# boqian333/E2ENet-Medical

Hardware: AMD Instinct MI355X
Metric: voxels/sec (train step fwd+bwd+update), 128^3 patch 32ch density=0.2 (higher is better)
Workload: dtype f32 (fp16x2 split products, f32 accumulate); 1 GPU; BraTS-shaped 4-modal 128^3 patches, shiftConvPP base 32, K=4, DSFF density 0.2, batch 2 per GPU, fwd+loss+bwd+clip+SGD+mask step, dense (parity) wgrad; parallelism=dp1

## Files before the change

e2enet_medical_amd/_lib.py:

```python
import ctypes as C
import os

_HERE = os.path.dirname(os.path.abspath(__file__))
LIB_PATH = os.environ.get("E2E_LIB_PATH") or os.path.join(_HERE, "csrc", "libe2e_hip.so")

KNOWN_ENV = frozenset({
    "E2E_CONV_MM", "E2E_MM_GRID", "E2E_MM_GEOM", "E2E_MM_PAIRQ", "E2E_CONV_DENSE", "E2E_CONV_SPARSE2", "E2E_CONV_PERSIST", "E2E_CONV_WGS",
    "E2E_CONV_KSPLIT", "E2E_WG_H2", "E2E_WG_BF3", "E2E_CT_BF3", "E2E_CT_H2",
    "E2E_CONV_DBG", "E2E_MM_STAMPS",
    "E2E_LIB_PATH", "E2E_STRICT_ENV", "E2E_DENSE_MIN_DENSITY", "E2E_MM_MIN_DENSITY", "E2E_WGRAD_STREAM", "E2E_LANES", "E2E_GRAPHS",
    "E2E_GRAPH_MAX_VOXELS", "E2E_PLAN_CACHE_GB", "E2E_SW_BLOCKING", "E2E_FORCE_DIST",
    "E2E_CPU_THREADS", "E2E_BENCH_DRY", "E2E_BENCH_DRY_FAIL_RANK", "E2E_BENCH_ALL_LAUNCHES",
})


def check_env(environ=None, strict=None):
    environ = os.environ if environ is None else environ
    unknown = sorted(k for k in environ if k.startswith("E2E_") and k not in KNOWN_ENV)
    if not unknown:
        return
    msg = ("unknown E2E_* environment variable(s) %s: not read by this build (known: %s)"
           % (", ".join(unknown), ", ".join(sorted(KNOWN_ENV))))
    if strict is None:
        strict = environ.get("E2E_STRICT_ENV") == "1"
    if strict:
        raise RuntimeError(msg)
    import warnings
    warnings.warn(msg + "; set E2E_STRICT_ENV=1 to refuse instead", RuntimeWarning, stacklevel=2)


class InChan(C.Structure):
    _fields_ = [("ptr", C.c_void_p), ("scale", C.c_void_p), ("shift", C.c_void_p),
                ("nstride", C.c_longlong), ("ab_nstride", C.c_int), ("dshift", C.c_int),
                ("slope", C.c_float), ("reserved", C.c_int)]


class OutChan(C.Structure):
    _fields_ = [("ptr", C.c_void_p), ("nstride", C.c_longlong), ("dshift", C.c_int), ("accumulate", C.c_int)]


class InSumChan(C.Structure):
    _fields_ = [("y", C.c_void_p), ("scale", C.c_void_p), ("shift", C.c_void_p), ("mean", C.c_void_p), ("rstd", C.c_void_p),
                ("part", C.c_void_p), ("nstride", C.c_longlong), ("part_nstride", C.c_longlong), ("ab_nstride", C.c_int),
                ("slope", C.c_float)]
# ... 33 lines not shown
    "e2e_last_error": (C.c_char_p, []),
    "e2e_abi_version": (I, []),
    "e2e_last_kernel": (C.c_char_p, []),
    "e2e_conv133_num_partials": (I, [I, I, I, I, I]),
    "e2e_conv133_fwd": (I, [P, I, P, P, P, P, P, I, I, I, I, I, I, I, I, P]),
    "e2e_conv133_fwd_ws_bytes": (LL, [I, I, I, I, I, I, I, I, I]),
    "e2e_conv133_fwd_splitk": (I, [P, I, P, P, P, P, P, I, I, I, I, I, I, I, I, P, LL, P]),
    "e2e_conv133_dgrad": (I, [P, P, P, P, I, I, I, I, I, I, I, I, I, P]),
    "e2e_conv133_dgrad_ws_bytes": (LL, [I, I, I, I, I, I, I, I, I]),
    "e2e_conv133_dgrad_splitk": (I, [P, P, P, P, I, I, I, I, I, I, I, I, I, P, LL, P]),
    "e2e_conv133_dense_ws_bytes": (LL, [I, I, I, I, I, I, I, I, I]),
    "e2e_conv133_sparse_eligible": (I, [I, I, I, I, I, I, I, I]),
    "e2e_conv133_sparse_wpk_floats": (LL, [I, I, I]),
    "e2e_conv133_sparse_plan": (I, [P, I, I, I, P, P, P, P, P, P]),
    "e2e_conv133_sparse_pack": (I, [P, I, LL, P]),
    "e2e_conv133_fwd_sparse": (I, [P, I, P, P, P, P, I, P, I, P, P, I, I, I, I, I, P]),
    "e2e_conv133_dgrad_sparse": (I, [P, P, P, P, I, P, P, P, I, I, I, I, I, I, I, P]),
    "e2e_conv133_fwd_dense": (I, [P, I, P, P, P, P, P, I, I, I, I, I, P, LL, P]),
    "e2e_conv133_mm_ws_bytes": (LL, [I, I, I, I, I, I, I, I, I]),
    "e2e_conv133_mm_pack": (I, [P, I, LL, P]),
    "e2e_conv133_input_ranges_ws_bytes": (LL, [I]),
    "e2e_conv133_input_ranges": (I, [P, I, P, P]),
    "e2e_absmax_word": (I, [P, LL, P, P]),
    "e2e_conv133_fwd_mm": (I, [P, I, P, P, P, P, P, P, I, I, I, I, I, P]),
    "e2e_conv133_dgrad_mm": (I, [P, P, P, P, P, I, I, I, I, I, I, P]),
    "e2e_conv133_dgrad_dense": (I, [P, P, P, P, I, I, I, I, I, I, P, LL, P]),
    "e2e_conv133_wgrad_ws_bytes": (LL, [I, I, I, I, I, I, I, I, I]),
    "e2e_conv133_wgrad": (I, [P, P, P, P, I, I, I, I, I, I, I, I, I, P, P, P]),
    "e2e_diag_split_gemm": (I, [P, P, P, I, I, P, P]),
    "e2e_diag_kernel_clock": (I, [I, P, P, I]),
    "e2e_in_stats_finalize": (I, [P, I, P, P, F, P, P, P, P, I, I, P]),
    "e2e_in_lrelu_bwd_ws_doubles": (LL, [I, I]),
    "e2e_in_lrelu_bwd": (I, [P, P, P, P, P, P, P, F, P, P, P, P, I, I, LL, P, I, P, P]),
    "e2e_convT_fwd": (I, [P, P, P, F, P, P, P, I, I, I, I, I, I, I, I, I, P, P, P]),
    "e2e_convT_dgrad": (I, [P, P, P, P, I, I, I, I, I, I, I, I, I, I, P, P, P, P]),
    "e2e_convT_wgrad_ws_bytes": (LL, [I, I, I, I, I, I, I, I, I]),
    "e2e_convT_wgrad": (I, [P, P, P, F, P, P, P, I, I, I, I, I, I, I, I, I, P, P, P, P]),
    "e2e_maxpool_fwd": (I, [P, P, P, F, P, I, I, I, I, I, I, I, I, P]),
    "e2e_maxpool_bwd_num_records": (I, [I, I, I, I, I, I]),
    "e2e_maxpool_bwd": (I, [P, P, P, F, P, P, I, I, I, I, I, I, I, I, I, P, P, P, P]),
    "e2e_head1x1_fwd": (I, [P, P, P, F, P, P, I, I, I, LL, P]),
    "e2e_head1x1_dgrad": (I, [P, P, P, I, I, I, I, LL, P]),
    "e2e_head1x1_wgrad_ws_bytes": (LL, [I, I, I, LL]),
    "e2e_head1x1_wgrad": (I, [P, P, P, F, P, P, P, I, I, I, LL, P]),
    "e2e_loss_ws_bytes": (LL, [I, I]),
    "e2e_dc_ce_reduce": (I, [P, P, P, I, I, LL, P]),
    "e2e_dc_ce_grad": (I, [P, P, P, F, I, F, P, P, I, I, LL, P]),
    "e2e_dc_ce_fold_batch": (I, [P, I, I, P]),
    "e2e_online_eval_counts": (I, [P, P, P, I, I, LL, P]),
    "e2e_dc_bce_reduce": (I, [P, P, P, P, I, I, LL, P]),
    "e2e_dc_bce_grad": (I, [P, P, P, P, F, I, F, P, P, I, I, LL, P]),
    "e2e_online_eval_regions": (I, [P, P, P, P, I, I, LL, P]),
    "e2e_seg_to_regions": (I, [P, P, P, I, I, LL, P]),
    "e2e_ds_target_gather": (I, [P, P, P, P, P, I, I, I, I, I, I, I, P]),
    "e2e_grad_sqnorm": (I, [P, I, P, P]),
    "e2e_sgd_clip_mask_step": (I, [P, I, P, F, F, F, F, I, I, P]),
    "e2e_apply_mask": (I, [P, I, P]),
    "e2e_dsff_kernel_l1": (I, [P, P, I, I, I, I, I, P]),
    "e2e_dsff_kth_value": (I, [P, I, I, P, P, P]),
    "e2e_dsff_death": (I, [P, P, P, I, P]),
    "e2e_dsff_grad_score": (I, [P, P, F, P, P, I, I, I, I, I, P]),
    "e2e_dsff_grow_above": (I, [P, P, P, I, I, I, P]),
    "e2e_dsff_expand": (I, [P, P, P, P, I, I, I, P]),
    "e2e_dsff_expand_quads": (I, [P, P, P, I, I, P]),
    "e2e_dsff_kmask_from_weights": (I, [P, P, I, I, I, P]),
    "e2e_flip3d": (I, [P, P, I, I, I, I, I, P]),
# ... 25 lines not shown


class _Lib:
    def __init__(self, path):
        if not os.path.exists(path):
            raise ImportError(
                "libe2e_hip.so not found at %s: build it with `python -c 'import __graft_entry__ as g; g.build()'` "
                "or `make -C e2enet_medical_amd/csrc`. There is no CPU fallback." % path)
        self._dll = C.CDLL(path)
        self.path = path
        for name, (res, args) in SIGNATURES.items():
            fn = getattr(self._dll, name)
            fn.restype = res
            fn.argtypes = args
            if name in _NO_STATUS:
                setattr(self, name[4:], fn)
            else:
                setattr(self, name[4:], self._checked(name, fn))

    def _checked(self, name, fn):
        last_error = self._dll.e2e_last_error

        def call(*a):
            rc = fn(*a)
            if rc != 0:
                raise E2EError("%s failed (%d): %s" % (name, rc, (last_error() or b"").decode()))
        call.__name__ = name
        return call


_lib = None


ABI_VERSION = 19


def lib() -> _Lib:
    global _lib
    if _lib is None:
        import torch
        check_env()
        handle = _Lib(LIB_PATH)
        got = handle.abi_version()
        if got != ABI_VERSION:
            raise ImportError("%s reports ABI version %d, this package needs %d: rebuild with `make -C %s`"
                              % (LIB_PATH, got, ABI_VERSION, os.path.dirname(LIB_PATH)))
        _lib = handle
    return _lib
```

e2enet_medical_amd/csrc/api.hip:

```cpp
#include "e2e_common.h"
#include <cstring>

namespace e2e {
static thread_local char g_err[512] = "";
void set_error(const char* fmt, ...) {
  va_list ap;
  va_start(ap, fmt);
  vsnprintf(g_err, sizeof(g_err), fmt, ap);
  va_end(ap);
}
static thread_local char g_kernel[160] = "";
void note_kernel(const char* fmt, ...) {
  va_list ap;
  va_start(ap, fmt);
  vsnprintf(g_kernel, sizeof(g_kernel), fmt, ap);
  va_end(ap);
}
}

extern "C" const char* e2e_last_error(void) { return e2e::g_err; }
extern "C" const char* e2e_last_kernel(void) { return e2e::g_kernel; }
extern "C" int e2e_abi_version(void) { return 19; }

extern "C" int e2e_diag_kernel_clock(int family, double* mhz, double* busy_ms, int reset) {
  E2E_REQUIRE(mhz != nullptr && (family == 0 || family == 1), "diag_kernel_clock: family 0 (conv133_mm) or 1 (conv133_wgrad v5)");
  if (hipDeviceSynchronize() != hipSuccess) return e2e::check_launch("diag_kernel_clock");
  unsigned long long v[2] = {0, 0};
  if (family == 0) e2e::mm_clock_read(v, reset != 0); else e2e::wgrad_clock_read(v, reset != 0);
  *mhz = v[1] ? 100.0 * (double)v[0] / (double)v[1] : 0.0;
  if (busy_ms) *busy_ms = (double)v[1] / 1e5;
  return e2e::check_launch("diag_kernel_clock");
}
```

e2enet_medical_amd/csrc/instnorm.hip:

```cpp
#include "e2e_common.h"
#include "e2e_split.h"

namespace {

struct Stat {
  double n, mean, m2;
};
__device__ __forceinline__ Stat combine(const Stat a, const Stat b) {
  if (b.n == 0.0) return a;
  if (a.n == 0.0) return b;
  Stat r;
  r.n = a.n + b.n;
  const double delta = b.mean - a.mean;
  r.mean = a.mean + delta * (b.n / r.n);
  r.m2 = a.m2 + b.m2 + delta * delta * (a.n * b.n / r.n);
  return r;
}

__global__ __launch_bounds__(256) void in_finalize_kernel(const double* __restrict__ part, int np,
                                                          const float* __restrict__ gamma,
                                                          const float* __restrict__ beta, float eps,
                                                          float* __restrict__ scale, float* __restrict__ shift,
                                                          float* __restrict__ mean_out, float* __restrict__ rstd_out,
                                                          int C) {
// ... 219 lines not shown
  const int c = blockIdx.x;
  double s3 = 0.0;
  if (dbias != nullptr) {
    for (int n = 0; n < B; ++n) {
      const double* q = rec3 + ((long long)n * C + c) * nblocks;
      for (int b = threadIdx.x; b < nblocks; b += 64) s3 += q[b];
    }
    s3 = e2e::wave_sum_d(s3);
  }
  if (threadIdx.x != 0) return;
  double s1 = 0.0, s2 = 0.0;
  for (int n = 0; n < B; ++n) {
    const double* r = sums + ((long long)n * C + c) * 3;
    s1 += r[0];
    s2 += r[1];
  }
  dbeta[c] = (float)s1;
  dgamma[c] = (float)s2;
  if (dbias) dbias[c] = (float)s3;
}

__global__ __launch_bounds__(64) void in_bwd_tile_sums_kernel(const double* __restrict__ part, double* __restrict__ sums, int np,
                                                              unsigned* __restrict__ absmax) {
  const int nc = blockIdx.x;
  if (absmax != nullptr && nc == 0 && threadIdx.x == 0) *absmax = 0u;
  const double* p = part + (long long)nc * np * 2;
  double a = 0.0, b = 0.0;
  for (int i = threadIdx.x; i < np; i += 64) { a += p[2 * i]; b += p[2 * i + 1]; }
  a = e2e::wave_sum_d(a);
  b = e2e::wave_sum_d(b);
  if (threadIdx.x == 0) { sums[(long long)nc * 3] = a; sums[(long long)nc * 3 + 1] = b; sums[(long long)nc * 3 + 2] = 0.0; }
}

}

extern "C" int e2e_in_stats_finalize(const double* part, int np, const float* gamma, const float* beta, float eps,
                                     float* scale, float* shift, float* mean, float* rstd, int B, int C,
                                     void* stream) {
  E2E_REQUIRE(part && gamma && beta && scale && shift && mean && rstd, "in_stats_finalize: null pointer");
  E2E_REQUIRE(np > 0 && B > 0 && C > 0, "in_stats_finalize: bad dims");
  hipLaunchKernelGGL(in_finalize_kernel, dim3(B * C), dim3(256), 0, (hipStream_t)stream, part, np, gamma, beta, eps,
                     scale, shift, mean, rstd, C);
  return e2e::check_launch("in_finalize_kernel");
}

extern "C" long long e2e_in_lrelu_bwd_ws_doubles(int B, int C) { return (long long)B * C * (3 + 3 * 256) + 2; }

extern "C" int e2e_in_lrelu_bwd(float* dz_dy, const float* y, const float* mean, const float* rstd, const float* scale,
                                const float* shift, const float* gamma, float slope, float* dgamma, float* dbeta,
                                float* dbias, float* sums, int B, int C, long long spatial, const double* tile_sums, int np,
                                unsigned* dy_absmax, void* stream) {
  E2E_REQUIRE(dz_dy && y && mean && rstd && scale && shift && gamma && dgamma && dbeta && sums, "in_lrelu_bwd: null pointer");
  E2E_REQUIRE(B > 0 && C > 0 && spatial > 0, "in_lrelu_bwd: bad dims");
  hipStream_t st = (hipStream_t)stream;
  double* ds = reinterpret_cast<double*>(sums);
  double* recs = ds + (long long)B * C * 3;
  double* rec3 = recs + (long long)B * C * 256 * 2;
  long long blocks = e2e::cdivll(spatial, 256 * 4 * 4);
  if (blocks > 256) blocks = 256;
  if (blocks < 1) blocks = 1;
  dim3 grid((unsigned)blocks, B * C);
  if (tile_sums == nullptr) {
    hipLaunchKernelGGL(in_bwd_reduce_kernel, grid, dim3(256), 0, st, dz_dy, y, mean, rstd, scale, shift, slope, recs, C,
                       spatial, dy_absmax, ds);
    hipLaunchKernelGGL(in_bwd_apply_kernel, grid, dim3(256), 0, st, dz_dy, y, mean, rstd, scale, shift, gamma, slope, ds,
                       (const double*)recs, (int)blocks, B, C, spatial, dy_absmax, rec3);
  } else {
    E2E_REQUIRE(np > 0, "in_lrelu_bwd: tile_sums without a record count");
    hipLaunchKernelGGL(in_bwd_tile_sums_kernel, dim3(B * C), dim3(64), 0, st, tile_sums, ds, np, dy_absmax);
    hipLaunchKernelGGL(in_bwd_apply_kernel, grid, dim3(256), 0, st, dz_dy, y, mean, rstd, scale, shift, gamma, slope, ds,
                       (const double*)nullptr, 0, B, C, spatial, dy_absmax, rec3);
  }
  hipLaunchKernelGGL(in_bwd_params_kernel, dim3(C), dim3(64), 0, st, (const double*)ds, (const double*)rec3, (int)blocks,
                     dgamma, dbeta, dbias, B, C);
  return e2e::check_launch("in_lrelu_bwd");
}
```

e2enet_medical_amd/engine.py:

```python
import contextlib
import ctypes as C
import math
import os
from typing import Dict, List, Optional, Sequence, Tuple

import torch

import numpy as np

from ._lib import lib, InChan, OutChan, ParamEntry, SparsePackJob, InSumChan, MmPackJob, RangeSrc, RangeJob

LRELU_SLOPE = 0.01
IN_EPS = 1e-5
DENSE_MIN_DENSITY = float(os.environ.get("E2E_DENSE_MIN_DENSITY", "0.5"))
WGRAD_STREAM = os.environ.get("E2E_WGRAD_STREAM", "1") != "0"
WGRAD_STREAM_MAX_ELEMS = 40000000
WGRAD_LATE = True
LANES = os.environ.get("E2E_LANES", "1") != "0"
LANE_DIVS = None


def _lane_divs(voxels):
    if LANE_DIVS is not None:
        return LANE_DIVS
    return (8, 512) if voxels <= (1 << 20) else (64,)
FUSE_IN_SUMS = 1
SPARSE2 = os.environ.get("E2E_CONV_SPARSE2", "1") != "0"
DENSE_ENABLED = True
MM_FORWARD = MM_BACKWARD = True
MM_MIN_DENSITY = float(os.environ.get("E2E_MM_MIN_DENSITY", "0.125"))


PARAM_EPOCH = 0


def note_native_param_write():
    global PARAM_EPOCH
    PARAM_EPOCH += 1


def shift_amounts(num_channels: int, shift_size: int = 5):
    group = math.ceil(num_channels / shift_size)
    pad = shift_size // 2
    return [c // group - pad for c in range(num_channels)]


def _stream():
    return torch.cuda.current_stream().cuda_stream


@contextlib.contextmanager
def _wgrad_stream(eng, elems):
    side = getattr(eng, "_wg_active", None)
    if side is None or elems > WGRAD_STREAM_MAX_ELEMS:
        yield eng.wgrad_ws
        return
    side.wait_stream(torch.cuda.current_stream())
    with torch.cuda.stream(side):
        yield eng.wgrad_ws_side


def _ptr(t: Optional[torch.Tensor]) -> int:
    return 0 if t is None else t.data_ptr()


def _upload_structs(structs, device) -> torch.Tensor:
    raw = b"".join(bytes(s) for s in structs)
    return torch.frombuffer(bytearray(raw), dtype=torch.uint8).to(device)


class Act:

    def __init__(self, name, shape, normed, device):
        self.name = name
        self.shape = tuple(int(v) for v in shape)
        self.normed = normed
        self.data = torch.empty(self.shape, dtype=torch.float32, device=device)
        b, c = self.shape[:2]
        if normed:
            self.scale = torch.empty(b * c, dtype=torch.float32, device=device)
            self.shift = torch.empty(b * c, dtype=torch.float32, device=device)
            self.mean = torch.empty(b * c, dtype=torch.float32, device=device)
            self.rstd = torch.empty(b * c, dtype=torch.float32, device=device)
        else:
            self.scale = self.shift = self.mean = self.rstd = None
        self.grad: Optional[torch.Tensor] = None
        self.needs_grad = True
        self._grad_written = False
        self.producer = None
        self.last_writer = None
        self.sums_ready = False

    @property
    def spatial(self):
        return self.shape[2] * self.shape[3] * self.shape[4]

    def alloc_grad(self):
        if self.grad is None and self.needs_grad:
            self.grad = torch.empty(self.shape, dtype=torch.float32, device=self.data.device)

    def claim_grad_write(self, op=None) -> int:
        acc = 1 if self._grad_written else 0
        self._grad_written = True
        self.last_writer = op
        return acc


class SparsePlan:

    def __init__(self, km_host, transpose, device):
        L = lib()
        r, cc = km_host.shape
        self.Q, self.P = (cc, r) if transpose else (r, cc)
        self.groups, self.nchunks = (self.Q + 31) // 32, (self.P + 7) // 8
        qslot = np.empty(self.groups * 32, dtype=np.int32)
        pslot = np.empty(self.groups * self.nchunks * 8, dtype=np.int32)
        quads = np.empty(self.groups * 8 * self.nchunks, dtype=np.uint32)
        woff = np.empty(self.groups * self.nchunks * 8, dtype=np.int32)
        flush, kmax = C.c_int(1), C.c_int(1)
        km_host = np.ascontiguousarray(km_host, dtype=np.uint8)
        L.conv133_sparse_plan(km_host.ctypes.data, r, cc, 1 if transpose else 0, qslot.ctypes.data, pslot.ctypes.data,
                              quads.ctypes.data, woff.ctypes.data, C.addressof(kmax), C.addressof(flush))
        self.flush_every, self.kmax = int(flush.value), int(kmax.value)
        self.woff = torch.from_numpy(woff).to(device)
# ... 225 lines not shown
        elif self.use_dense():
            L.conv133_fwd_dense(self.chans.data_ptr(), self.cin, p[self.w_name].data_ptr(), p[self.prefix + ".conv.bias"].data_ptr(),
                                _ptr(self.live), self.out.data.data_ptr(), self.part.data_ptr(), b, self.cout, di, hi, wi, ws.data_ptr(),
                                ws.numel() * 4, _stream())
        elif self.sp_fwd is not None:
            sp = self.sp_fwd
            L.conv133_fwd_sparse(sp.table.data_ptr(), self.cin, sp.wpk.data_ptr(), p[self.prefix + ".conv.bias"].data_ptr(),
                                 sp.quads.data_ptr(), sp.woff.data_ptr(), sp.kmax, sp.qslot.data_ptr(), sp.flush_every, self.out.data.data_ptr(),
                                 self.part.data_ptr(), b, self.cout, di, hi, wi, _stream())
        elif ws is not None and self.fwd_ws_bytes > 0:
            L.conv133_fwd_splitk(self.chans.data_ptr(), self.cin, p[self.w_name].data_ptr(),
                                 p[self.prefix + ".conv.bias"].data_ptr(), _ptr(self.live), self.out.data.data_ptr(),
                                 self.part.data_ptr(), b, self.cout, di, hi, wi, sd, sh, sw, ws.data_ptr(), ws.numel() * 4,
                                 _stream())
        else:
            L.conv133_fwd(self.chans.data_ptr(), self.cin, p[self.w_name].data_ptr(), p[self.prefix + ".conv.bias"].data_ptr(),
                          _ptr(self.live), self.out.data.data_ptr(), self.part.data_ptr(), b, self.cout, di, hi, wi,
                          sd, sh, sw, _stream())
        L.in_stats_finalize(self.part.data_ptr(), self.np, p[self.prefix + ".instnorm.weight"].data_ptr(),
                            p[self.prefix + ".instnorm.bias"].data_ptr(), IN_EPS, self.out.scale.data_ptr(),
                            self.out.shift.data_ptr(), self.out.mean.data_ptr(), self.out.rstd.data_ptr(), b,
                            self.cout, _stream())

    def backward(self):
        e = self.eng
        p, g = e.params, e.grads
        o = self.out
        b = o.shape[0]
        di, hi, wi = self.in_dims
        sd, sh, sw = self.stride
        L = lib()
        ready = o.sums_ready
        o.sums_ready = False
        L.in_lrelu_bwd(o.grad.data_ptr(), o.data.data_ptr(), o.mean.data_ptr(), o.rstd.data_ptr(), o.scale.data_ptr(), o.shift.data_ptr(),
                       p[self.prefix + ".instnorm.weight"].data_ptr(),
                       LRELU_SLOPE, g[self.prefix + ".instnorm.weight"].data_ptr(),
                       g[self.prefix + ".instnorm.bias"].data_ptr(), g[self.prefix + ".conv.bias"].data_ptr(),
                       e.in_sums.data_ptr(), b, self.cout, o.spatial, self.own_sums.data_ptr() if ready else None, self.own_np,
                       self.dy_absmax.data_ptr(), _stream())
        late = WGRAD_LATE and getattr(e, "_wg_active", None) is not None and o.data.numel() > WGRAD_STREAM_MAX_ELEMS
        if not late:
            self._wgrad(e, L, g, o, b, di, hi, wi, sd, sh, sw, o.data.numel())
        if self.do_dgrad:
            ws = getattr(e, "fwd_ws", None)
            if self.use_mm("b"):
                if not hasattr(e, "_refresh_weight_caches"):
                    self.pack_mm_standalone("b")
                L.conv133_dgrad_mm(o.grad.data_ptr(), self.dy_absmax.data_ptr(), self.wpk_bwd.data_ptr(), self.w_absmax.data_ptr(),
                                   self.outs.data_ptr(), b, self.cin, self.cout, di, hi, wi, _stream())
            elif self.use_dense():
                L.conv133_dgrad_dense(o.grad.data_ptr(), p[self.w_name].data_ptr(), _ptr(self.live_t), self.outs.data_ptr(), b, self.cin, self.cout,
                                      di, hi, wi, ws.data_ptr(), ws.numel() * 4, _stream())
            elif self.sp_bwd is not None:
                sp = self.sp_bwd
                table = self._bwd_table()
                L.conv133_dgrad_sparse(o.grad.data_ptr(), sp.wpk.data_ptr(), sp.quads.data_ptr(), sp.woff.data_ptr(), sp.kmax, sp.pslot.data_ptr(),
                                       table.data_ptr(), _ptr(sp.insum), sp.flush_every, b, self.cin, self.cout, di, hi, wi, _stream())
                for s in sp.fused_srcs:
                    s.sums_ready = True
            elif ws is not None and self.dgrad_ws_bytes > 0:
                L.conv133_dgrad_splitk(o.grad.data_ptr(), p[self.w_name].data_ptr(), _ptr(self.live_t), self.outs.data_ptr(),
                                       b, self.cin, self.cout, di, hi, wi, sd, sh, sw, ws.data_ptr(), ws.numel() * 4, _stream())
            else:
                L.conv133_dgrad(o.grad.data_ptr(), p[self.w_name].data_ptr(), _ptr(self.live_t), self.outs.data_ptr(),
                                b, self.cin, self.cout, di, hi, wi, sd, sh, sw, _stream())
        if late:
            self._wgrad(e, L, g, o, b, di, hi, wi, sd, sh, sw, 0)

    def _wgrad(self, e, L, g, o, b, di, hi, wi, sd, sh, sw, elems):
        with _wgrad_stream(e, elems) as ws:
            L.conv133_wgrad(self.chans.data_ptr(), o.grad.data_ptr(), g[self.w_name].data_ptr(), ws.data_ptr(),
                            b, self.cin, self.cout, di, hi, wi, sd, sh, sw, self.dy_absmax.data_ptr(), self.x_absmax_ptr(), _stream())
# ... 111 lines not shown
        self.out.pool_of = src.producer if src.normed else None
        self.acc = 0

    def plan_backward(self):
        self.src.alloc_grad()
        self.acc = self.src.claim_grad_write(self)

    def forward(self):
        s = self.src
        b, c, d, h, w = s.shape
        lib().maxpool_fwd(s.data.data_ptr(), _ptr(s.scale), _ptr(s.shift), LRELU_SLOPE, self.out.data.data_ptr(),
                          b, c, d, h, w, *self.kernel, _stream())

    def backward(self):
        s = self.src
        b, c, d, h, w = s.shape
        fuse = FUSE_IN_SUMS >= 1 and s.normed and s.last_writer is self and s.producer is not None and s.producer.own_sums is not None
        lib().maxpool_bwd(s.data.data_ptr(), _ptr(s.scale), _ptr(s.shift), LRELU_SLOPE, self.out.grad.data_ptr(),
                          s.grad.data_ptr(), self.acc, b, c, d, h, w, *self.kernel,
                          s.mean.data_ptr() if fuse else None, s.rstd.data_ptr() if fuse else None,
                          s.producer.own_sums.data_ptr() if fuse else None, _stream())
        if fuse:
            s.sums_ready = True


class HeadOp:

    def __init__(self, eng, w_name, src: Act, num_classes):
        self.eng, self.w_name, self.src, self.k = eng, w_name, src, num_classes
        b, c = src.shape[:2]
        self.out = Act(w_name, (b, num_classes) + src.shape[2:], False, eng.device)
        self.acc = 0
        self.active = True

    def plan_backward(self):
        self.src.alloc_grad()
        self.acc = self.src.claim_grad_write(self)

    def forward(self):
        s = self.src
        b, c = s.shape[:2]
        lib().head1x1_fwd(s.data.data_ptr(), _ptr(s.scale), _ptr(s.shift), LRELU_SLOPE,
                          self.eng.params[self.w_name].data_ptr(), self.out.data.data_ptr(), b, c, self.k, s.spatial,
                          _stream())

    def backward(self):
        s, e = self.src, self.eng
        b, c = s.shape[:2]
        L = lib()
        with _wgrad_stream(e, s.data.numel()) as ws:
            L.head1x1_wgrad(s.data.data_ptr(), _ptr(s.scale), _ptr(s.shift), LRELU_SLOPE, self.out.grad.data_ptr(),
                            e.grads[self.w_name].data_ptr(), ws.data_ptr(), b, c, self.k, s.spatial, _stream())
        L.head1x1_dgrad(self.out.grad.data_ptr(), e.params[self.w_name].data_ptr(), s.grad.data_ptr(), self.acc, b, c,
                        self.k, s.spatial, _stream())


class NetConfig:

    def __init__(self, in_channels, base_features, num_classes, pool_kernels, convs_per_stage=2, max_features=320,
                 shift_size=5, graph="unetpp"):
        if graph not in ("unetpp", "unet"):
            raise ValueError("graph must be 'unetpp' (unetpp_d.py) or 'unet' (unetpp_d_nodff.py)")
        self.graph = graph
        if graph == "unetpp" and len(pool_kernels) != 5:
            raise ValueError("shiftConvPP needs exactly 5 pooling stages, got %d" % len(pool_kernels))
        self.in_channels, self.base_features, self.num_classes = in_channels, base_features, num_classes
        self.pool_kernels = [tuple(int(v) for v in k) for k in pool_kernels]
        self.convs_per_stage, self.max_features = convs_per_stage, max_features
        if shift_size < 1 or shift_size % 2 == 0:
            raise ValueError("shift_size must be odd and >= 1 (reference unetpp_d.py:89 uses 5; 1 disables the shift)")
        self.shift_size = shift_size
        feats, f = [], base_features
        for _ in range(len(pool_kernels) + 1):
            feats.append(min(f, max_features))
            f = min(int(round(f * 2)), max_features)
        self.feats = feats

    @property
    def num_pool(self):
        return len(self.pool_kernels)

    def nest_nodes(self, z):
        k = self.num_pool - z
        return [(m, k - 1 - m) for m in range(k)]

# ... 265 lines not shown

    def _plan_lanes(self):
        vox = self.patch[0] * self.patch[1] * self.patch[2]
        self._lane_of = [sum(1 for dv in self.lane_divs if op.out.spatial * dv <= vox) for op in self.ops]
        writer = {}
        self._deps_fwd = []
        for i, op in enumerate(self.ops):
            self._deps_fwd.append(sorted({writer[id(a)] for a in self._reads(op)
                                          if id(a) in writer and self._lane_of[writer[id(a)]] != self._lane_of[i]}))
            writer[id(op.out)] = i
        self._ev_fwd = self._events_for(self._deps_fwd)
        self._deps_bwd, self._ev_bwd = None, None
        self._lane_streams = None

    def _backward_order(self):
        order = list(reversed(range(len(self.ops))))
        if FUSE_IN_SUMS < 1:
            return order
        index = {id(op): i for i, op in enumerate(self.ops)}
        for i, op in enumerate(self.ops):
            prod = getattr(op.src, "producer", None) if isinstance(op, PoolOp) else None
            if prod is None or id(prod) not in index:
                continue
            order.remove(i)
            order.insert(order.index(index[id(prod)]), i)
        return order

    def _plan_lanes_backward(self):
        last = {}
        self._deps_bwd = [None] * len(self.ops)
        for i in self._bwd_order:
            op = self.ops[i]
            touched = [op.out] + [a for a in self._reads(op) if a.grad is not None]
            self._deps_bwd[i] = sorted({last[id(a)] for a in touched
                                        if id(a) in last and self._lane_of[last[id(a)]] != self._lane_of[i]})
            for a in touched:
                last[id(a)] = i
        self._ev_bwd = self._events_for(self._deps_bwd)

    @staticmethod
    def _events_for(deps):
        return {j: None for d in deps for j in d}

    def _lanes_on(self):
        return LANES and any(self._lane_of) and not self._graph_ok() and not torch.cuda.is_current_stream_capturing()

    def _exec(self, order, deps, events, action, checkpoint=None):
        main = torch.cuda.current_stream()
        if not self._lanes_on():
            for i in order:
                action(self.ops[i])
                if checkpoint is not None:
                    checkpoint(self.ops[i], lambda st: st.wait_stream(main))
            return
        if self._lane_streams is None:
            self._lane_streams = [torch.cuda.Stream(device=self.device) for _ in self.lane_divs]
        side = self._lane_streams
        streams = [main] + side

        def join():
            for st in side:
                main.wait_stream(st)

        def wait_all(st):
            for s_ in streams:
                st.wait_stream(s_)
# ... 23 lines not shown

    def _graph_ok(self):
        mode = os.environ.get("E2E_GRAPHS", "auto")
        if mode == "0" or self.grad_bucket_hook is not None or self.batch_dice_hook is not None:
            return False
        if torch.cuda.is_current_stream_capturing():
            return False
        if mode == "1":
            return True
        if LANES and self.lane_divs:
            return False
        vox = self.batch * self.patch[0] * self.patch[1] * self.patch[2]
        return vox <= int(os.environ.get("E2E_GRAPH_MAX_VOXELS", str(1 << 20)))

    def _run(self, key, fn):
        if not self._graph_ok():
            return fn()
        key = key + (self.maps_generation,)
        g = self._graphs.get(key)
        if g is None:
            if key not in self._graph_seen:
                self._graph_seen.add(key)
                return fn()
            g = torch.cuda.CUDAGraph()
            torch.cuda.synchronize()
            with torch.cuda.graph(g):
                fn()
            self._graphs[key] = g
        g.replay()

    def prepare_backward(self):
        if self._backward_ready:
            return
        for op in (self.ops[i] for i in self._bwd_order):
            op.out.alloc_grad()
            op.plan_backward()
        order, seen = [], set()
        for op in (self.ops[i] for i in self._bwd_order):
            if isinstance(op, ConvOp):
                produced = [op.w_name, op.prefix + ".conv.bias", op.prefix + ".instnorm.weight", op.prefix + ".instnorm.bias"]
            elif isinstance(op, (UpOp, HeadOp)):
                produced = [op.w_name]
            else:
                produced = []
            for name in produced:
                if name in self.params and name not in seen:
                    order.append((name, op))
                    seen.add(name)
        order += [(name, None) for name in self.params if name not in seen]
        offs, total = {}, 0
        for name, _ in order:
            offs[name] = total
            total += (self.params[name].numel() + 63) // 64 * 64
        self.grad_flat = torch.zeros(total, dtype=torch.float32, device=self.device)
        for name, p in self.params.items():
            self.grads[name] = self.grad_flat[offs[name]:offs[name] + p.numel()].view(p.shape)
        self._bucket_after_op, lo, nb = {}, 0, 4
        for i, (name, op) in enumerate(order):
            end = offs[name] + (self.params[name].numel() + 63) // 64 * 64
            last_of_op = i + 1 == len(order) or order[i + 1][1] is not op
            if op is not None and last_of_op and (end - lo >= total // nb):
                self._bucket_after_op[id(op)] = (lo, end)
                lo = end
        self._bucket_tail = (lo, total)
        ws = max([op.wgrad_ws_bytes() for op in self.ops if hasattr(op, "wgrad_ws_bytes")] +
                 [lib().head1x1_wgrad_ws_bytes(self.batch, h.src.shape[1], h.k, h.src.spatial) for h in self.heads])
        self._wgrad_ws = [torch.empty((ws + 3) // 4, dtype=torch.float32, device=self.device) for _ in range(len(self.lane_divs) + 1)]
        cmax = max(op.cout for op in self.conv_ops.values())
        self._in_sums = [torch.zeros(int(lib().in_lrelu_bwd_ws_doubles(self.batch, cmax)), dtype=torch.float64, device=self.device)
                         for _ in range(len(self.lane_divs) + 1)]
        for op in self.conv_ops.values():
            d_, h_, w_ = op.out_dims
            lw = op.out.last_writer
            op.own_sums, op.own_np = None, 0
            if isinstance(lw, PoolOp) and FUSE_IN_SUMS >= 1:
                op.own_np = int(lib().maxpool_bwd_num_records(d_, h_, w_, *lw.kernel))
            elif isinstance(lw, ConvOp) and FUSE_IN_SUMS >= 2 and lw.sparse_ok:
                op.own_np = d_ * ((h_ + 15) // 16) * ((w_ + 31) // 32)
            if op.own_np > 0:
                op.own_sums = torch.zeros(self.batch * op.cout * op.own_np * 2, dtype=torch.float64, device=self.device)
            if op.sp_bwd is not None:
                op.sp_bwd.table = None
        self._plan_lanes_backward()
        self._loss_buffers()
        self._backward_ready = True

    def backward(self, dlogits: Optional[Sequence[Optional[torch.Tensor]]] = None):
        self.prepare_backward()
        if dlogits is not None:
            for h, g in zip(self.heads, dlogits):
                if g is None:
                    h.out.grad.zero_()
                else:
                    h.out.grad.copy_(g)
        for op in self.conv_ops.values():
            op.out.sums_ready = False
        self._refresh_weight_caches("b")
        hook = self.grad_bucket_hook
        main = torch.cuda.current_stream()
        if WGRAD_STREAM and not self._graph_ok() and not torch.cuda.is_current_stream_capturing():
            if self._wg_side is None:
                self._wg_side = torch.cuda.Stream(device=self.device)
                self.wgrad_ws_side = torch.empty_like(self._wgrad_ws[0])
            self._wg_active = self._wg_side
        side = self._wg_active

        def act(op):
            if isinstance(op, HeadOp) and not op.active:
                if op.acc == 0:
                    op.src.grad.zero_()
                self.grads[op.w_name].zero_()
            else:
                op.backward()

        def checkpoint(op, wait_all):
            if hook is not None and id(op) in self._bucket_after_op:
                if self._comm_stream is None:
                    self._comm_stream = torch.cuda.Stream(device=self.device)
                comm = self._comm_stream
# ... 125 lines not shown
```

include/e2e_hip.h:

```cpp
#ifndef E2E_HIP_H
#define E2E_HIP_H

#ifdef __cplusplus
extern "C" {
#endif

#define E2E_OK 0
#define E2E_ERR_ARG (-1)
#define E2E_ERR_LAUNCH (-2)
#define E2E_ERR_UNSUPPORTED (-3)

const char* e2e_last_error(void);
int e2e_abi_version(void);
const char* e2e_last_kernel(void);

typedef struct {
  const float* ptr;
  const float* scale;
  const float* shift;
  long long nstride;
  int ab_nstride;
  int dshift;
  float slope;
  int reserved;
// ... 83 lines not shown
  int wCout, wks;
  const unsigned* word;
} e2e_range_src_t;
typedef struct {
  e2e_range_src_t src[3];
  unsigned* out;
} e2e_range_job_t;
long long e2e_conv133_mm_ws_bytes(int B, int Cin, int Cout, int Di, int Hi, int Wi, int sd, int sh, int sw);
int e2e_conv133_mm_pack(const e2e_mm_pack_job_t* jobs, int njobs, long long max_elems, void* stream);
long long e2e_conv133_input_ranges_ws_bytes(int njobs);
int e2e_conv133_input_ranges(const e2e_range_job_t* jobs, int njobs, void* ws, void* stream);
int e2e_absmax_word(const float* x, long long n, unsigned* word, void* stream);
int e2e_conv133_fwd_mm(const e2e_in_chan_t* chans, int Cin, const void* wpk, const unsigned* w_absmax, const float* bias,
                       const unsigned* x_absmax, float* y, double* part, int B, int Cout, int Di, int Hi, int Wi, void* stream);
int e2e_conv133_dgrad_mm(const float* dy, const unsigned* dy_absmax, const void* wpk_t, const unsigned* w_absmax,
                         const e2e_out_chan_t* outs, int B, int Cin, int Cout, int Di, int Hi, int Wi, void* stream);

long long e2e_conv133_wgrad_ws_bytes(int B, int Cin, int Cout, int Di, int Hi, int Wi, int sd, int sh, int sw);
int e2e_conv133_wgrad(const e2e_in_chan_t* chans, const float* dy, float* dw, void* ws, int B, int Cin,
                      int Cout, int Di, int Hi, int Wi, int sd, int sh, int sw, const unsigned* dy_absmax,
                      const unsigned* x_absmax, void* stream);

int e2e_diag_split_gemm(const float* A, const float* Bt, float* D, int K, int mode, const unsigned* absmax_b, void* stream);

int e2e_diag_kernel_clock(int family, double* mhz, double* busy_ms, int reset);

int e2e_in_stats_finalize(const double* part, int np, const float* gamma, const float* beta, float eps,
                          float* scale, float* shift, float* mean, float* rstd, int B, int C, void* stream);

long long e2e_in_lrelu_bwd_ws_doubles(int B, int C);
int e2e_in_lrelu_bwd(float* dz_dy, const float* y, const float* mean, const float* rstd, const float* scale, const float* shift,
                     const float* gamma, float slope, float* dgamma, float* dbeta, float* dbias, float* sums,
                     int B, int C, long long spatial, const double* tile_sums, int np, unsigned* dy_absmax, void* stream);

int e2e_convT_fwd(const float* x, const float* scale, const float* shift, float slope, const float* w,
                  const unsigned* live, float* y, int B, int Cin, int Cout, int D, int H, int W, int kd,
                  int kh, int kw, const unsigned* x_absmax, const unsigned* w_absmax, void* stream);
int e2e_convT_dgrad(const float* dy, const float* w, const unsigned* live_t, float* dx, int accumulate, int B,
                    int Cin, int Cout, int D, int H, int W, int kd, int kh, int kw, const unsigned* w_absmax,
                    const unsigned* dy_bound_a, const unsigned* dy_bound_b, void* stream);
long long e2e_convT_wgrad_ws_bytes(int B, int Cin, int Cout, int D, int H, int W, int kd, int kh, int kw);
int e2e_convT_wgrad(const float* x, const float* scale, const float* shift, float slope, const float* dy,
                    float* dw, void* ws, int B, int Cin, int Cout, int D, int H, int W, int kd, int kh, int kw,
                    const unsigned* x_absmax, const unsigned* dy_bound_a, const unsigned* dy_bound_b, void* stream);

int e2e_maxpool_fwd(const float* x, const float* scale, const float* shift, float slope, float* y, int B, int C,
                    int D, int H, int W, int kd, int kh, int kw, void* stream);
int e2e_maxpool_bwd_num_records(int D, int H, int W, int kd, int kh, int kw);
int e2e_maxpool_bwd(const float* x, const float* scale, const float* shift, float slope, const float* dy,
                    float* dx, int accumulate, int B, int C, int D, int H, int W, int kd, int kh, int kw,
                    const float* mean, const float* rstd, double* tile_sums, void* stream);

int e2e_head1x1_fwd(const float* x, const float* scale, const float* shift, float slope, const float* w,
                    float* logits, int B, int C, int K, long long spatial, void* stream);
int e2e_head1x1_dgrad(const float* dlogits, const float* w, float* dx, int accumulate, int B, int C, int K,
                      long long spatial, void* stream);
long long e2e_head1x1_wgrad_ws_bytes(int B, int C, int K, long long spatial);
int e2e_head1x1_wgrad(const float* x, const float* scale, const float* shift, float slope,
                      const float* dlogits, float* dw, void* ws, int B, int C, int K, long long spatial,
                      void* stream);

long long e2e_loss_ws_bytes(int B, int K);
int e2e_dc_ce_reduce(const float* logits, const float* target, void* acc, int B, int K, long long spatial,
                     void* stream);
int e2e_dc_ce_grad(const float* logits, const float* target, const void* acc, float weight, int batch_dice,
                   float smooth, float* dlogits, float* loss_out, int B, int K, long long spatial, void* stream);
// ... 85 lines not shown
```

Before: 129.5 million voxels/s.

## Fold 1x1 head dgrad into instance-norm LeakyReLU backward kernels

When a segmentation head reads a normed activation with at most one other consumer, the head's input-gradient (a K-term weighted sum of dlogits) is computed on the fly inside the instance-norm backward reduce and apply kernels. This replaces the separate head1x1_dgrad launch and avoids materialising and re-reading that gradient at full resolution. In exchange, dlogits is read twice (once per pass), an extra K loads per element are added, and the backward dependency graph must track the head output.

Result: no change. 129.9 million voxels/s (median of 6 runs) (+0.4%).

```diff
diff --git a/e2enet_medical_amd/_lib.py b/e2enet_medical_amd/_lib.py
--- a/e2enet_medical_amd/_lib.py
+++ b/e2enet_medical_amd/_lib.py
@@ -9,7 +9,7 @@
     "E2E_CONV_KSPLIT", "E2E_WG_H2", "E2E_WG_BF3", "E2E_CT_BF3", "E2E_CT_H2",
     "E2E_CONV_DBG", "E2E_MM_STAMPS",
     "E2E_LIB_PATH", "E2E_STRICT_ENV", "E2E_DENSE_MIN_DENSITY", "E2E_MM_MIN_DENSITY", "E2E_WGRAD_STREAM", "E2E_LANES", "E2E_GRAPHS",
-    "E2E_GRAPH_MAX_VOXELS", "E2E_PLAN_CACHE_GB", "E2E_SW_BLOCKING", "E2E_FORCE_DIST",
+    "E2E_GRAPH_MAX_VOXELS", "E2E_FOLD_BWD", "E2E_PLAN_CACHE_GB", "E2E_SW_BLOCKING", "E2E_FORCE_DIST",
     "E2E_CPU_THREADS", "E2E_BENCH_DRY", "E2E_BENCH_DRY_FAIL_RANK", "E2E_BENCH_ALL_LAUNCHES",
 })
 
@@ -109,6 +109,7 @@
     "e2e_in_stats_finalize": (I, [P, I, P, P, F, P, P, P, P, I, I, P]),
     "e2e_in_lrelu_bwd_ws_doubles": (LL, [I, I]),
     "e2e_in_lrelu_bwd": (I, [P, P, P, P, P, P, P, F, P, P, P, P, I, I, LL, P, I, P, P]),
+    "e2e_in_lrelu_bwd_head": (I, [P, P, P, P, P, P, P, F, P, P, P, P, I, I, LL, P, P, P, I, I, P]),
     "e2e_convT_fwd": (I, [P, P, P, F, P, P, P, I, I, I, I, I, I, I, I, I, P, P, P]),
     "e2e_convT_dgrad": (I, [P, P, P, P, I, I, I, I, I, I, I, I, I, I, P, P, P, P]),
     "e2e_convT_wgrad_ws_bytes": (LL, [I, I, I, I, I, I, I, I, I]),
@@ -200,7 +201,7 @@
 _lib = None
 
 
-ABI_VERSION = 19
+ABI_VERSION = 20
 
 
 def lib() -> _Lib:
diff --git a/e2enet_medical_amd/csrc/api.hip b/e2enet_medical_amd/csrc/api.hip
--- a/e2enet_medical_amd/csrc/api.hip
+++ b/e2enet_medical_amd/csrc/api.hip
@@ -20,7 +20,7 @@
 
 extern "C" const char* e2e_last_error(void) { return e2e::g_err; }
 extern "C" const char* e2e_last_kernel(void) { return e2e::g_kernel; }
-extern "C" int e2e_abi_version(void) { return 19; }
+extern "C" int e2e_abi_version(void) { return 20; }
 
 extern "C" int e2e_diag_kernel_clock(int family, double* mhz, double* busy_ms, int reset) {
   E2E_REQUIRE(mhz != nullptr && (family == 0 || family == 1), "diag_kernel_clock: family 0 (conv133_mm) or 1 (conv133_wgrad v5)");
diff --git a/e2enet_medical_amd/csrc/instnorm.hip b/e2enet_medical_amd/csrc/instnorm.hip
--- a/e2enet_medical_amd/csrc/instnorm.hip
+++ b/e2enet_medical_amd/csrc/instnorm.hip
@@ -275,6 +275,197 @@
   if (threadIdx.x == 0) { sums[(long long)nc * 3] = a; sums[(long long)nc * 3 + 1] = b; sums[(long long)nc * 3 + 2] = 0.0; }
 }
 
+struct FoldBlock {
+  int bx, nc, c, n;
+};
+__device__ __forceinline__ FoldBlock fold_block(int nb, int C) {
+  FoldBlock f;
+  f.c = (int)blockIdx.x % C;
+  const int pair = (int)blockIdx.x / C;
+  f.bx = pair % nb;
+  f.n = pair / nb;
+  f.nc = f.n * C + f.c;
+  return f;
+}
+
+template <int KB, bool HAS_DZ>
+__device__ __forceinline__ e2e::f32x4_t head_dz(const float* __restrict__ dlp, long long spatial, long long i, const float (&wk)[KB],
+                                                int K, const float* __restrict__ dzp) {
+#pragma clang fp contract(off)
+  e2e::f32x4_t g[KB];
+#pragma unroll
+  for (int k = 0; k < KB; ++k) g[k] = IN_LD(dlp + (long long)(k < K ? k : 0) * spatial + i);
+  float s[4] = {0.f, 0.f, 0.f, 0.f};
+#pragma unroll
+  for (int k = 0; k < KB; ++k)
+#pragma unroll
+    for (int j = 0; j < 4; ++j) s[j] = k < K ? fmaf(wk[k], g[k][j], s[j]) : s[j];
+  e2e::f32x4_t o = {s[0], s[1], s[2], s[3]};
+  if (HAS_DZ) {
+    const e2e::f32x4_t t = IN_LD(dzp + i);
+#pragma unroll
+    for (int j = 0; j < 4; ++j) o[j] += t[j];
+  }
+  return o;
+}
+
+template <int KB, bool HAS_DZ>
+__global__ __launch_bounds__(256) void in_bwd_reduce_head_kernel(const float* __restrict__ dz, const float* __restrict__ y,
+                                                                 const float* __restrict__ mean, const float* __restrict__ rstd,
+                                                                 const float* __restrict__ scale, const float* __restrict__ shift,
+                                                                 float slope, double* __restrict__ recs, int nb, int B, int C,
+                                                                 long long spatial, unsigned* __restrict__ absmax,
+                                                                 double* __restrict__ s3_zero, const float* __restrict__ dl,
+                                                                 const float* __restrict__ hw, int K) {
+#pragma clang fp contract(off)
+  const FoldBlock f = fold_block(nb, C);
+  const int nc = f.nc;
+  if (absmax != nullptr && f.bx == 0 && nc == 0 && threadIdx.x == 0) *absmax = 0u;
+  if (f.bx == 0 && threadIdx.x == 0) s3_zero[(long long)nc * 3 + 2] = 0.0;
+  const float mu = mean[nc], rs = rstd[nc], sca = scale[nc], shf = shift[nc];
+  float wk[KB];
+#pragma unroll
+  for (int k = 0; k < KB; ++k) wk[k] = k < K ? hw[(long long)k * C + f.c] : 0.f;
+  const float* dzp = dz + (long long)nc * spatial;
+  const float* yp = y + (long long)nc * spatial;
+  const float* dlp = dl + (long long)f.n * K * spatial;
+  float s1 = 0.f, s2 = 0.f;
+  double d1 = 0.0, d2 = 0.0;
+  const long long stride = (long long)nb * 256 * 4;
+  int it = 0;
+  for (long long i = ((long long)f.bx * 256 + threadIdx.x) * 4; i < spatial; i += stride) {
+    const e2e::f32x4_t dv = head_dz<KB, HAS_DZ>(dlp, spatial, i, wk, K, dzp);
+    const e2e::f32x4_t yv = IN_LD(yp + i);
+#pragma unroll
+    for (int k = 0; k < 4; ++k) {
+      const float xh = (yv[k] - mu) * rs;
+      const float u = fmaf(yv[k], sca, shf);
+      const float du = u > 0.f ? dv[k] : dv[k] * slope;
+      s1 += du;
+      s2 = fmaf(du, xh, s2);
+    }
+    if ((++it & 15) == 0) {
+      d1 += s1; d2 += s2; s1 = 0.f; s2 = 0.f;
+    }
+  }
+  d1 += s1; d2 += s2;
+  d1 = e2e::wave_sum_d(d1);
+  d2 = e2e::wave_sum_d(d2);
+  __shared__ double sh[2][4];
+  const int wave = threadIdx.x >> 6, lane = threadIdx.x & 63;
+  if (lane == 0) { sh[0][wave] = d1; sh[1][wave] = d2; }
+  __syncthreads();
+  if (threadIdx.x == 0) {
+    double* r = recs + ((long long)nc * nb + f.bx) * 2;
+    r[0] = sh[0][0] + sh[0][1] + sh[0][2] + sh[0][3];
+    r[1] = sh[1][0] + sh[1][1] + sh[1][2] + sh[1][3];
+  }
+}
+
+template <int KB, bool HAS_DZ>
+__global__ __launch_bounds__(256) void in_bwd_apply_head_kernel(float* __restrict__ dz, const float* __restrict__ y,
+                                                                const float* __restrict__ mean, const float* __restrict__ rstd,
+                                                                const float* __restrict__ scale, const float* __restrict__ shift,
+                                                                const float* __restrict__ gamma, float slope,
+                                                                double* __restrict__ sums, const double* __restrict__ rec, int nb,
+                                                                int B, int C, long long spatial, unsigned* __restrict__ absmax,
+                                                                double* __restrict__ rec3, const float* __restrict__ dl,
+                                                                const float* __restrict__ hw, int K) {
+#pragma clang fp contract(off)
+  const FoldBlock f = fold_block(nb, C);
+  const int nc = f.nc;
+  const float mu = mean[nc], rs = rstd[nc], g = gamma[f.c], sca = scale[nc], shf = shift[nc];
+  float wk[KB];
+#pragma unroll
+  for (int k = 0; k < KB; ++k) wk[k] = k < K ? hw[(long long)k * C + f.c] : 0.f;
+  __shared__ double s12[2];
+  if (threadIdx.x < 64) {
+    const double* r = rec + (long long)nc * nb * 2;
+    double a = 0.0, b = 0.0;
+    for (int i = threadIdx.x; i < nb; i += 64) { a += r[2 * i]; b += r[2 * i + 1]; }
+    a = e2e::wave_sum_d(a);
+    b = e2e::wave_sum_d(b);
+    if (threadIdx.x == 0) {
+      s12[0] = a; s12[1] = b;
+      if (f.bx == 0) { sums[(long long)nc * 3] = a; sums[(long long)nc * 3 + 1] = b; }
+    }
+  }
+  __syncthreads();
+  const double inv_n = 1.0 / (double)spatial;
+  const float m1 = (float)(s12[0] * inv_n);
+  const float m2 = (float)(s12[1] * inv_n);
+  const float grs = g * rs;
+  float* dzp = dz + (long long)nc * spatial;
+  const float* yp = y + (long long)nc * spatial;
+  const float* dlp = dl + (long long)f.n * K * spatial;
+  double acc = 0.0;
+  float amax = 0.f;
+  const long long stride = (long long)nb * 256 * 4;
+  long long i = ((long long)f.bx * 256 + threadIdx.x) * 4;
+  for (; i + stride < spatial; i += 2 * stride) {
+    const e2e::f32x4_t a0 = head_dz<KB, HAS_DZ>(dlp, spatial, i, wk, K, dzp), q0 = IN_LDY(yp + i);
+    const e2e::f32x4_t a1 = head_dz<KB, HAS_DZ>(dlp, spatial, i + stride, wk, K, dzp), q1 = IN_LDY(yp + i + stride);
+    e2e::f32x4_t o0, o1;
+    float part0 = 0.f, part1 = 0.f;
+#pragma unroll
+    for (int k = 0; k < 4; ++k) {
+      const float xh0 = (q0[k] - mu) * rs, xh1 = (q1[k] - mu) * rs;
+      const float u0 = fmaf(q0[k], sca, shf), u1 = fmaf(q1[k], sca, shf);
+      const float du0 = u0 > 0.f ? a0[k] : a0[k] * slope, du1 = u1 > 0.f ? a1[k] : a1[k] * slope;
+      const float t0 = fmaf(-xh0, m2, du0 - m1), t1 = fmaf(-xh1, m2, du1 - m1);
+      o0[k] = grs * t0;
+      o1[k] = grs * t1;
+      part0 = fmaf(grs, t0, part0);
+      part1 = fmaf(grs, t1, part1);
+      amax = fmaxf(amax, fmaxf(fabsf(o0[k]), fabsf(o1[k])));
+    }
+    acc += part0;
+    acc += part1;
+    *reinterpret_cast<e2e::f32x4_t*>(dzp + i) = o0;
+    *reinterpret_cast<e2e::f32x4_t*>(dzp + i + stride) = o1;
+  }
+  for (; i < spatial; i += stride) {
+    const e2e::f32x4_t a = head_dz<KB, HAS_DZ>(dlp, spatial, i, wk, K, dzp);
+    const e2e::f32x4_t q = IN_LDY(yp + i);
+    e2e::f32x4_t o;
+    float part = 0.f;
+#pragma unroll
+    for (int k = 0; k < 4; ++k) {
+      const float xh = (q[k] - mu) * rs;
+      const float u = fmaf(q[k], sca, shf);
+      const float du = u > 0.f ? a[k] : a[k] * slope;
+      o[k] = grs * fmaf(-xh, m2, du - m1);
+      part += o[k];
+      amax = fmaxf(amax, fabsf(o[k]));
+    }
+    acc += part;
+    *reinterpret_cast<e2e::f32x4_t*>(dzp + i) = o;
+  }
+  acc = e2e::wave_sum_d(acc);
+#pragma unroll
+  for (int off = 32; off > 0; off >>= 1) amax = fmaxf(amax, __shfl_xor(amax, off, 64));
+  __shared__ double sh[4];
+  __shared__ float shm[4];
+  const int wave = threadIdx.x >> 6, lane = threadIdx.x & 63;
+  if (lane == 0) { sh[wave] = acc; shm[wave] = amax; }
+  __syncthreads();
+  if (threadIdx.x == 0) {
+    rec3[(long long)nc * nb + f.bx] = sh[0] + sh[1] + sh[2] + sh[3];
+    if (absmax != nullptr) atomicMax(absmax, __builtin_bit_cast(unsigned, fmaxf(fmaxf(shm[0], shm[1]), fmaxf(shm[2], shm[3]))));
+  }
+}
+
+template <int KB, bool HAS_DZ>
+void launch_head_fold(hipStream_t st, int nb, float* dz_dy, const float* y, const float* mean, const float* rstd, const float* scale,
+                      const float* shift, const float* gamma, float slope, double* ds, double* recs, double* rec3, int B, int C,
+                      long long spatial, unsigned* dy_absmax, const float* dl, const float* hw, int K) {
+  const dim3 grid((unsigned)(nb * B * C));
+  hipLaunchKernelGGL((in_bwd_reduce_head_kernel<KB, HAS_DZ>), grid, dim3(256), 0, st, (const float*)dz_dy, y, mean, rstd, scale, shift,
+                     slope, recs, nb, B, C, spatial, dy_absmax, ds, dl, hw, K);
+  hipLaunchKernelGGL((in_bwd_apply_head_kernel<KB, HAS_DZ>), grid, dim3(256), 0, st, dz_dy, y, mean, rstd, scale, shift, gamma, slope,
+                     ds, (const double*)recs, nb, B, C, spatial, dy_absmax, rec3, dl, hw, K);
+}
+
 }
 
 extern "C" int e2e_in_stats_finalize(const double* part, int np, const float* gamma, const float* beta, float eps,
@@ -318,3 +509,40 @@
                      dgamma, dbeta, dbias, B, C);
   return e2e::check_launch("in_lrelu_bwd");
 }
+
+extern "C" int e2e_in_lrelu_bwd_head(float* dz_dy, const float* y, const float* mean, const float* rstd, const float* scale,
+                                     const float* shift, const float* gamma, float slope, float* dgamma, float* dbeta,
+                                     float* dbias, float* sums, int B, int C, long long spatial, unsigned* dy_absmax,
+                                     const float* dlogits, const float* head_w, int K, int has_dz, void* stream) {
+  E2E_REQUIRE(dz_dy && y && mean && rstd && scale && shift && gamma && dgamma && dbeta && sums && dlogits && head_w,
+              "in_lrelu_bwd_head: null pointer");
+  E2E_REQUIRE(B > 0 && C > 0 && spatial > 0 && K > 0, "in_lrelu_bwd_head: bad dims");
+  if (spatial % 4 != 0 || K > 16) {
+    e2e::set_error("in_lrelu_bwd_head: needs spatial %% 4 == 0 and K <= 16 (spatial %lld, K %d): materialise with e2e_head1x1_dgrad",
+                   spatial, K);
+    return E2E_ERR_UNSUPPORTED;
+  }
+  hipStream_t st = (hipStream_t)stream;
+  double* ds = reinterpret_cast<double*>(sums);
+  double* recs = ds + (long long)B * C * 3;
+  double* rec3 = recs + (long long)B * C * 256 * 2;
+  long long blocks = e2e::cdivll(spatial, 256 * 4 * 4);
+  if (blocks > 256) blocks = 256;
+  if (blocks < 1) blocks = 1;
+  E2E_REQUIRE(blocks * B * C < (1ll << 30), "in_lrelu_bwd_head: too many (n, c) planes");
+  const int nb = (int)blocks;
+#define FOLD_LAUNCH(KB)                                                                                                          \
+  do {                                                                                                                           \
+    if (has_dz) launch_head_fold<KB, true>(st, nb, dz_dy, y, mean, rstd, scale, shift, gamma, slope, ds, recs, rec3, B, C,       \
+                                           spatial, dy_absmax, dlogits, head_w, K);                                             \
+    else launch_head_fold<KB, false>(st, nb, dz_dy, y, mean, rstd, scale, shift, gamma, slope, ds, recs, rec3, B, C, spatial,    \
+                                     dy_absmax, dlogits, head_w, K);                                                             \
+  } while (0)
+  if (K <= 4) FOLD_LAUNCH(4);
+  else if (K <= 8) FOLD_LAUNCH(8);
+  else FOLD_LAUNCH(16);
+#undef FOLD_LAUNCH
+  hipLaunchKernelGGL(in_bwd_params_kernel, dim3(C), dim3(64), 0, st, (const double*)ds, (const double*)rec3, nb, dgamma, dbeta,
+                     dbias, B, C);
+  return e2e::check_launch("in_lrelu_bwd_head");
+}
diff --git a/e2enet_medical_amd/engine.py b/e2enet_medical_amd/engine.py
--- a/e2enet_medical_amd/engine.py
+++ b/e2enet_medical_amd/engine.py
@@ -25,6 +25,7 @@
         return LANE_DIVS
     return (8, 512) if voxels <= (1 << 20) else (64,)
 FUSE_IN_SUMS = 1
+FOLD_BWD = os.environ.get("E2E_FOLD_BWD", "1") != "0"
 SPARSE2 = os.environ.get("E2E_CONV_SPARSE2", "1") != "0"
 DENSE_ENABLED = True
 MM_FORWARD = MM_BACKWARD = True
@@ -90,6 +91,7 @@
         self.producer = None
         self.last_writer = None
         self.sums_ready = False
+        self.head_term = None
 
     @property
     def spatial(self):
@@ -381,12 +383,21 @@
         L = lib()
         ready = o.sums_ready
         o.sums_ready = False
-        L.in_lrelu_bwd(o.grad.data_ptr(), o.data.data_ptr(), o.mean.data_ptr(), o.rstd.data_ptr(), o.scale.data_ptr(), o.shift.data_ptr(),
-                       p[self.prefix + ".instnorm.weight"].data_ptr(),
-                       LRELU_SLOPE, g[self.prefix + ".instnorm.weight"].data_ptr(),
-                       g[self.prefix + ".instnorm.bias"].data_ptr(), g[self.prefix + ".conv.bias"].data_ptr(),
-                       e.in_sums.data_ptr(), b, self.cout, o.spatial, self.own_sums.data_ptr() if ready else None, self.own_np,
-                       self.dy_absmax.data_ptr(), _stream())
+        head = o.head_term
+        if head is not None and head.active:
+            L.in_lrelu_bwd_head(o.grad.data_ptr(), o.data.data_ptr(), o.mean.data_ptr(), o.rstd.data_ptr(), o.scale.data_ptr(),
+                                o.shift.data_ptr(), p[self.prefix + ".instnorm.weight"].data_ptr(), LRELU_SLOPE,
+                                g[self.prefix + ".instnorm.weight"].data_ptr(), g[self.prefix + ".instnorm.bias"].data_ptr(),
+                                g[self.prefix + ".conv.bias"].data_ptr(), e.in_sums.data_ptr(), b, self.cout, o.spatial,
+                                self.dy_absmax.data_ptr(), head.out.grad.data_ptr(), p[head.w_name].data_ptr(), head.k, head.acc,
+                                _stream())
+        else:
+            L.in_lrelu_bwd(o.grad.data_ptr(), o.data.data_ptr(), o.mean.data_ptr(), o.rstd.data_ptr(), o.scale.data_ptr(), o.shift.data_ptr(),
+                           p[self.prefix + ".instnorm.weight"].data_ptr(),
+                           LRELU_SLOPE, g[self.prefix + ".instnorm.weight"].data_ptr(),
+                           g[self.prefix + ".instnorm.bias"].data_ptr(), g[self.prefix + ".conv.bias"].data_ptr(),
+                           e.in_sums.data_ptr(), b, self.cout, o.spatial, self.own_sums.data_ptr() if ready else None, self.own_np,
+                           self.dy_absmax.data_ptr(), _stream())
         late = WGRAD_LATE and getattr(e, "_wg_active", None) is not None and o.data.numel() > WGRAD_STREAM_MAX_ELEMS
         if not late:
             self._wgrad(e, L, g, o, b, di, hi, wi, sd, sh, sw, o.data.numel())
@@ -564,10 +575,12 @@
         self.out = Act(w_name, (b, num_classes) + src.shape[2:], False, eng.device)
         self.acc = 0
         self.active = True
+        self.fold = False
 
     def plan_backward(self):
         self.src.alloc_grad()
-        self.acc = self.src.claim_grad_write(self)
+        if not self.fold:
+            self.acc = self.src.claim_grad_write(self)
 
     def forward(self):
         s = self.src
@@ -583,6 +596,8 @@
         with _wgrad_stream(e, s.data.numel()) as ws:
             L.head1x1_wgrad(s.data.data_ptr(), _ptr(s.scale), _ptr(s.shift), LRELU_SLOPE, self.out.grad.data_ptr(),
                             e.grads[self.w_name].data_ptr(), ws.data_ptr(), b, c, self.k, s.spatial, _stream())
+        if self.fold:
+            return
         L.head1x1_dgrad(self.out.grad.data_ptr(), e.params[self.w_name].data_ptr(), s.grad.data_ptr(), self.acc, b, c,
                         self.k, s.spatial, _stream())
 
@@ -914,6 +929,8 @@
         for i in self._bwd_order:
             op = self.ops[i]
             touched = [op.out] + [a for a in self._reads(op) if a.grad is not None]
+            if op.out.head_term is not None:
+                touched.append(op.out.head_term.out)
             self._deps_bwd[i] = sorted({last[id(a)] for a in touched
                                         if id(a) in last and self._lane_of[last[id(a)]] != self._lane_of[i]})
             for a in touched:
@@ -1003,9 +1020,15 @@
     def prepare_backward(self):
         if self._backward_ready:
             return
+        for h in self.heads:
+            h.fold = FOLD_BWD and self._head_folds(h)
+            h.src.head_term = h if h.fold else None
         for op in (self.ops[i] for i in self._bwd_order):
             op.out.alloc_grad()
             op.plan_backward()
+        for h in self.heads:
+            if h.fold:
+                h.acc = 1 if h.src._grad_written else 0
         order, seen = [], set()
         for op in (self.ops[i] for i in self._bwd_order):
             if isinstance(op, ConvOp):
@@ -1056,6 +1079,17 @@
         self._loss_buffers()
         self._backward_ready = True
 
+    def _head_folds(self, h):
+        s = h.src
+        if not (s.normed and s.needs_grad and s.producer is not None and any(op is s.producer for op in self.ops)):
+            return False
+        if s.spatial % 4 != 0 or h.k > 16:
+            return False
+        others = [op for op in self.ops if op is not h and any(a is s for a in self._reads(op))]
+        if len(others) > 1 or any(isinstance(op, (PoolOp, HeadOp)) for op in others):
+            return False
+        return FUSE_IN_SUMS < 2 or not any(isinstance(op, ConvOp) for op in others)
+
     def backward(self, dlogits: Optional[Sequence[Optional[torch.Tensor]]] = None):
         self.prepare_backward()
         if dlogits is not None:
diff --git a/include/e2e_hip.h b/include/e2e_hip.h
--- a/include/e2e_hip.h
+++ b/include/e2e_hip.h
@@ -139,6 +139,10 @@
 int e2e_in_lrelu_bwd(float* dz_dy, const float* y, const float* mean, const float* rstd, const float* scale, const float* shift,
                      const float* gamma, float slope, float* dgamma, float* dbeta, float* dbias, float* sums,
                      int B, int C, long long spatial, const double* tile_sums, int np, unsigned* dy_absmax, void* stream);
+int e2e_in_lrelu_bwd_head(float* dz_dy, const float* y, const float* mean, const float* rstd, const float* scale, const float* shift,
+                          const float* gamma, float slope, float* dgamma, float* dbeta, float* dbias, float* sums,
+                          int B, int C, long long spatial, unsigned* dy_absmax, const float* dlogits, const float* head_w,
+                          int K, int has_dz, void* stream);
 
 int e2e_convT_fwd(const float* x, const float* scale, const float* shift, float slope, const float* w,
                   const unsigned* live, float* y, int B, int Cin, int Cout, int D, int H, int W, int kd,
```
